# wjwei-handsome/wgatools

Hardware: AMD Instinct MI355X
Metric: paf_cigar_ops_per_s (paf2maf+stat) (higher is better)
Workload: dtype u8

## Files before the change

wgatools_amd/csrc/wga_kernels_k2s.h:

```cpp
#ifndef WGA_KERNELS_K2S_H
#define WGA_KERNELS_K2S_H

#include "wga_kernels.h"

#define WGA_S_FIFO 320u
#define WGA_S_MAX_TILE_COLS (1ull << 24)
#define WGA_S_MAX_JOB_TILES 32u
#define WGA_S_SKIP 0x100u
#define WGA_S_U 4u
#define WGA_S_WAVE_BYTES ((WGA_S_FIFO + 4u) * 8u + 1024u + 1024u + 256u + 272u + 16u)
#ifndef WGA_AUTO_LONG_VARIANT
#define WGA_AUTO_LONG_VARIANT 3
#endif

__global__ __launch_bounds__(256) void k_stream_mark_rec(u32 n, const wga_rec_desc* recs, const u64* op_off, u64 t_fa_bytes,
                                                         u64 q_fa_bytes, u8* tile_flag) {
  const u32 r = blockIdx.x * 256u + threadIdx.x;
  if (r >= n) return;
  const wga_rec_desc d = recs[r];
  const bool inside = d.t_src_off >= 32ull && d.t_src_off + d.t_src_len + 32ull <= t_fa_bytes && d.q_src_off >= 32ull &&
                      d.q_src_off + d.q_src_len + 32ull <= q_fa_bytes;
  if ((d.neg & 0xEull) == 0ull && inside) return;
  const u64 a = op_off[r], b = op_off[r + 1];
  if (b <= a) return;
// ... 29 lines not shown
  d.q_src_len = q_src_len ? q_src_len[r] : 0ull;
  d.I_total = cs.i + cs.s;
  d.D_total = cs.d;
  d.L = cs.mx + cs.d;
  const bool clean = !q_src_len || d.q_src_len == cs.mx + cs.i + cs.s;
  const bool inside = !q_src_off || (d.q_src_off >= 32ull && d.q_src_off + d.q_src_len + 32ull <= q_fa_bytes);
  d.neg = (strand_neg[r] != 0 ? 1u : 0u) | (clean ? 0u : 8u);
  out[r] = d;
  if (clean && inside) return;
  const u64 a = op_off[r], b = op_off[r + 1];
  if (b <= a) return;
  for (u64 t = a / WGA_TILE; t <= (b - 1) / WGA_TILE; t++) tile_flag[t] = 1;
}

__device__ __forceinline__ u32 comp4s(u32 x, u32* bad) {
  const u32 sel = x & 0x07070707u;
  const u32 fold = byte_perm(0x474EFF54u, 0x43FF41FFu, sel);
  const u32 comp = byte_perm(0x434E0D41u, 0x47FF54FFu, sel);
  *bad = (x & 0xDFDFDFDFu) ^ fold;
  return comp | (x & 0x20202020u);
}

#define WGA_S_NOINLINE __forceinline__
__device__ WGA_S_NOINLINE void stream_store_bytes(u8* p, u32 o0, u32 o1, u32 o2, u32 o3, int lo, int hi) {
#pragma clang loop vectorize(disable) unroll(disable)
  for (int j = lo; j < hi; j++) {
    const u32 wj = j < 4 ? o0 : j < 8 ? o1 : j < 12 ? o2 : o3;
    p[j] = (u8)(wj >> (8 * (j & 3)));
  }
}
__device__ WGA_S_NOINLINE void stream_report_bad(u64* bad_base_pos, u32 b0, u32 b1, u32 b2, u32 b3, int lo, int hi, u32 Cl,
                                                 i64 Kseg, const u32* fifo, u32 k, u32 nf, u32 adj) {
#pragma clang loop vectorize(disable) unroll(disable)
  for (int j = lo; j < hi; j++) {
    const u32 bw = j < 4 ? b0 : j < 8 ? b1 : j < 12 ? b2 : b3;
    if (((bw >> (8 * (j & 3))) & 0xFFu) == 0u) continue;
    const u32 cj = Cl + (u32)j;
    u32 ad = adj;
    if (fifo) {
      u32 i = k - 1u;
      while (i + 1u < nf && (int)(fifo[2u * (i + 1u)] - cj) <= 0) i++;
      ad = fifo[2u * (i + 1u) + 1u];
    }
    atomicMin(bad_base_pos, (u64)((i64)(u64)(cj - ad) + Kseg));
  }
}
// ... 55 lines not shown
    u32 n_new = nf;
    if (lane == 0u) {
      u32 w = e0;
      for (u32 r = e0; r < nf; r++) {
        const u32 gs = s_fifo[2u * r], cu = s_fifo[2u * r + 1u];
        const bool dup = w > e0 && s_fifo[2u * (w - 1u)] == gs && (int)(cu - s_fifo[2u * (w - 1u) + 1u]) <= 0 &&
                         (int)(s_fifo[2u * (r + 1u) + 1u] - cu) <= 0;
        if (!dup) {
          s_fifo[2u * w] = gs;
          s_fifo[2u * w + 1u] = cu;
          w++;
        }
      }
      for (u32 k = 0; k < 3u; k++) {
        s_fifo[2u * (w + k)] = s_fifo[2u * (nf + k)];
        s_fifo[2u * (w + k) + 1u] = s_fifo[2u * (nf + k) + 1u];
      }
      n_new = w;
    }
    nf = wave_get_u32(n_new, 0);
    WGA_WAVE_SYNC();
  };

  for (;;) {
    {
      const u32 lim = bnd ? C_b : C_known;
      const bool all = bnd || fin;
      while ((int)(lim - pos) > 0) {
        if (TCOORD && (int)(C_min - pos) > 0) {
          const u32 to = (int)(lim - C_min) > 0 ? C_min : lim;
          u32 c;
          do {
            const u32 idx = e0 + lane < nf ? e0 + lane : nf;
            c = (u32)__popcll(__ballot(idx < nf && (int)(s_fifo[2u * idx] - to) < 0));
            e0 += c;
          } while (c == 64u);
          pos = to;
          continue;
        }
        u8* const A = dst_seg + pos;
        const u32 mis = (u32)(u64)A & 1023u;
        u8* const B = A - mis;
        const u32 room = WGA_S_U * 1024u - mis;
        if (!all && (lim - pos) < room) break;
        const u32 Cs = pos;
        u32 Ce = (lim - pos) < room ? lim : pos + room;
        const u32 Cl0 = Cs - mis;
        if (e0 + 255u < nf) {
          const u32 g255 = WGA_UNI32(s_fifo[2u * (e0 + 255u)]);
          if ((int)(g255 - Ce) < 0) Ce = Cl0 + ((g255 - Cl0) & ~15u);
          if (MODE == WGA_S_PSEUDO && (int)(Ce - Cs) < 16) {
            fifo_dedupe();
            continue;
          }
        }

        s_T[lane] = 0u;
        WGA_WAVE_SYNC();
        u32 nE = 0;
        {
          u32 base = e0, c;
          do {
            const u32 idx = base + lane < nf ? base + lane : nf;
            const u32 gsr = s_fifo[2u * idx] - Cl0;
            const bool in = gsr < Ce - Cl0;
            c = (u32)__popcll(__ballot(in));
            if (in) atomicAdd(&s_T[(gsr >> 4) & 63u], 1u << (8u * (gsr >> 10)));
            base += c;
            nE += c;
          } while (c == 64u);
        }
        WGA_WAVE_SYNC();
        const u32 tw = s_T[lane];
        WGA_WAVE_SYNC();
        const u32 tinc = wave_incl_scan_u32(tw);
        const u32 texc = tinc - tw;
        const u32 ttot = wave_last_u32(tinc);

        u32 kbase = e0;
        u32 qn = 0, rpk = 0, cls = 0;
        u32 adjv[WGA_S_U];
        const u32 wsp = Ce - Cs - 16u, asp = Ce - Cs + 15u;
        const bool any16 = (Ce - Cs) >= 16u;
        u32 qcum = 0;
#pragma unroll
        for (u32 u = 0; u < WGA_S_U; u++) {
          const u32 cnt = (tw >> (8u * u)) & 255u;
          const u32 k = kbase + ((texc >> (8u * u)) & 255u);
          kbase += (ttot >> (8u * u)) & 255u;
          const u32 Cl = Cl0 + 1024u * u + 16u * lane;
          const bool whole = any16 && (Cl - Cs) <= wsp, active = (Cl + 15u - Cs) < asp;
          const u32x4_a1 fe = *(const u32x4_a1*)(s_fifo + 2u * (k - 1u));
          const int rel0 = (int)(fe[0] + stream_glen<MODE>(fe[1], fe[3]) - Cl);
          const bool quiet = whole && cnt == 0u;
          const bool plain = quiet && rel0 <= 0;
          const bool dashes = quiet && rel0 >= 16;
          const bool flagged = active && !(plain || dashes);
          adjv[u] = fe[3];
          cls |= ((plain ? 1u : 0u) | (dashes ? 2u : 0u) | (flagged ? 4u : 0u) | (SYM ? (fe[1] & 1u) << 3 : 0u)) << (4u * u);
          const u64 m = __ballot(flagged);
          if (flagged) {
            const u32 r = qn + lane_rank(m, lane);
            s_q[r & 255u] = (k << 8) | (u << 6) | lane;
            rpk |= (r & 255u) << (8u * u);
          }
          qcum |= (qn > 255u ? 255u : qn) << (8u * u);
          qn += (u32)__popcll(m);
        }
        if (qn > 64u) {
          u32 keep = 1u;
#pragma unroll
          for (u32 u = 2; u <= WGA_S_U; u++) {
            const u32 upto = u == WGA_S_U ? qn : (qcum >> (8u * u)) & 255u;
            const bool sat = u < WGA_S_U && ((qcum >> (8u * u)) & 255u) == 255u;
            if (upto <= 64u && !sat) keep = u;
          }
          const u32 Cn = Cl0 + 1024u * keep;
          if ((int)(Cn - Ce) < 0) Ce = Cn;
          qn = keep == WGA_S_U ? qn : (qcum >> (8u * keep)) & 255u;
          nE = 0;
#pragma unroll
          for (u32 u = 0; u < WGA_S_U; u++)
            if (u < keep) nE += (ttot >> (8u * u)) & 255u;
        }
        const BufRsrc dbuf = buf_make(B, WGA_S_U * 1024u);

        WGA_WAVE_SYNC();
        if (lane < qn) {
          const u32 ent = s_q[lane];
          const u32 k = ent >> 8, Cl = Cl0 + 16u * (ent & 255u);
          int lo = (int)(Cs - Cl), hi = (int)(Ce - Cl);
          lo = lo < 0 ? 0 : (lo > 16 ? 16 : lo);
          hi = hi > 16 ? 16 : (hi < 0 ? 0 : hi);
          const u32x4_a1 ea = *(const u32x4_a1*)(s_fifo + 2u * (k - 1u));
          const u32x4_a1 eb = *(const u32x4_a1*)(s_fifo + 2u * (k + 1u));
          const u32 gs0 = ea[0], cu0 = ea[1], gs1 = ea[2], cu1 = ea[3], gs2 = eb[0], cu2 = eb[1];
          int a1 = (int)(gs0 + stream_glen<MODE>(cu0, cu1) - Cl);
          a1 = a1 < lo ? lo : (a1 > hi ? hi : a1);
          int b1 = (int)(gs1 - Cl);
          b1 = b1 < a1 ? a1 : (b1 > hi ? hi : b1);
          const u32 gl1 = stream_glen<MODE>(cu1, cu2);
          int e1 = gl1 >= 16u ? 16 : b1 + (int)gl1;
          e1 = e1 > hi ? hi : e1;
          bool more = (int)(gs2 - Cl) < hi;
          u32 W0[4], W1[4];
          if (!SYM) {
            buf_load16(sbuf, b1 > a1 ? (rc ? S32 - Cl + cu1 : S32 + Cl - cu1) : WGA_BUF_OOB, W0);
            buf_load16(sbuf, hi > e1 ? (rc ? S32 - Cl + cu2 : S32 + Cl - cu2) : WGA_BUF_OOB, W1);
          }
          const u32x4_a16 La = s_lm[a1], Lb = s_lm[b1], Le = s_lm[e1];
          u32 o[4], bad[4] = {0u, 0u, 0u, 0u};
#pragma unroll
          for (int d = 0; d < 4; d++) {
            if (SYM) {
              o[d] = bfi_b32(La[d], stream_symbol(cu0), bfi_b32(Le[d] & ~Lb[d], stream_symbol(cu1), 0x31313131u));
              continue;
            }
            u32 cp;
            if (rc)
              cp = comp4s(bfi_b32(Lb[d], bswap32(W0[3 - d]), bswap32(W1[3 - d])), &bad[d]);
            else
              cp = bfi_b32(Lb[d], W0[d], W1[d]);
            const u32 md = La[d] | (Le[d] & ~Lb[d]);
            o[d] = bfi_b32(md, 0x2D2D2D2Du, cp);
            bad[d] &= ~md;
          }
          u32 ie = k + 1u;
          while (more) {
            const u32 gsi = s_fifo[2u * ie], cui = s_fifo[2u * ie + 1u], gsn = s_fifo[2u * ie + 2u], cun = s_fifo[2u * ie + 3u];
            const int b = (int)(gsi - Cl);
            const u32 len = stream_glen<MODE>(cui, cun);
            const int e = len >= (u32)(hi - b) ? hi : b + (int)len;
            u32 W[4];
            if (SYM)
              W[0] = W[1] = W[2] = W[3] = 0x31313131u;
            else
              buf_load16(sbuf, rc ? S32 - Cl + cun : S32 + Cl - cun, W);
            const u32x4_a16 Mb = s_lm[b], Me = s_lm[e];
#pragma unroll
            for (int d = 0; d < 4; d++) {
              u32 x = W[d], bw = 0u;
              if (rc) x = comp4s(bswap32(W[3 - d]), &bw);
              if (SYM)
                o[d] = bfi_b32(Mb[d], o[d], bfi_b32(Me[d], stream_symbol(cui), x));
              else
                o[d] = bfi_b32(Mb[d], o[d], bfi_b32(Me[d], 0x2D2D2D2Du, x));
              bad[d] = (bad[d] & Mb[d]) | (bw & ~Me[d]);
            }
            ie++;
            more = (int)(gsn - Cl) < hi;
          }
          if (rc && (bad[0] | bad[1] | bad[2] | bad[3]) != 0u)
            stream_report_bad((u64*)&a.diag[rec].bad_base_pos, bad[0], bad[1], bad[2], bad[3], lo, hi, Cl, (i64)s_k[0], s_fifo, k, nf, 0u);
          const u32x4_a16 ov = {o[0], o[1], o[2], o[3]};
          s_P[lane] = ov;
        }
        WGA_WAVE_SYNC();

        u32 dat[WGA_S_U][4];
        const u32 wsp2 = Ce - Cs - 16u;
#pragma unroll
        for (u32 u = 0; u < WGA_S_U; u++) {
          const u32 Cl = Cl0 + 1024u * u + 16u * lane;
          const u32 c = (cls >> (4u * u)) & 15u;
          if (SYM) {
            dat[u][0] = dat[u][1] = dat[u][2] = dat[u][3] = (c & 2u) ? ((c & 8u) ? 0x2D2D2D2Du : 0x30303030u) : 0x31313131u;
            continue;
          }
          dat[u][0] = dat[u][1] = dat[u][2] = dat[u][3] = (c & 2u) ? 0x2D2D2D2Du : 0u;
          if ((c & 1u) && (int)(Cl - Ce) < 0) buf_load16(sbuf, rc ? S32 - Cl + adjv[u] : S32 + Cl - adjv[u], dat[u]);
        }
        if (rc) {
#pragma unroll
          for (u32 u = 0; u < WGA_S_U; u++) {
            u32 bad[4], x[4];
#pragma unroll
            for (int d = 0; d < 4; d++) x[d] = comp4s(bswap32(dat[u][3 - d]), &bad[d]);
#pragma unroll
            for (int d = 0; d < 4; d++) dat[u][d] = x[d];
            const u32 Cl = Cl0 + 1024u * u + 16u * lane;
            const bool pb = ((cls >> (4u * u)) & 1u) != 0u && (int)(Cl - Ce) < 0 && (bad[0] | bad[1] | bad[2] | bad[3]) != 0u;
            if (__ballot(pb)) {
              if (pb)
                stream_report_bad((u64*)&a.diag[rec].bad_base_pos, bad[0], bad[1], bad[2], bad[3], 0, 16, Cl, (i64)s_k[0], nullptr, 0u, 0u,
                                  adjv[u]);
            }
          }
        }
#pragma unroll
        for (u32 u = 0; u < WGA_S_U; u++) {
          const u32 Cl = Cl0 + 1024u * u + 16u * lane;
          const bool queued = ((cls >> (4u * u)) & 4u) != 0u && (int)(Cl - Ce) < 0;
          if (queued) {
            const u32x4_a16 pv = s_P[(rpk >> (8u * u)) & 255u];
            dat[u][0] = pv[0];
            dat[u][1] = pv[1];
            dat[u][2] = pv[2];
            dat[u][3] = pv[3];
          }
          const bool whole = (Ce - Cs) >= 16u && (Cl - Cs) <= wsp2;
          buf_store16_stream(dbuf, whole ? 1024u * u + 16u * lane : WGA_BUF_OOB, dat[u]);
          if (queued && !whole) {
            int lo = (int)(Cs - Cl), hi = (int)(Ce - Cl);
            lo = lo < 0 ? 0 : lo;
            hi = hi > 16 ? 16 : hi;
            stream_store_bytes(B + 1024u * u + lane * 16u, dat[u][0], dat[u][1], dat[u][2], dat[u][3], lo, hi);
          }
        }
        WGA_WAVE_SYNC();
        e0 += nE;
        pos = Ce;
      }
      fin = false;
    }

    if (bnd || !live) {
      const bool sw = bnd;
      u64 row_off, src_off, src_len, x_a, sb;
      bool neg;
      u32 C_a, cum_a;
      if (bnd) {
        const u64 bnd_op = job_lo + re;
        u64 ren;
        do {
          rec++;
          ren = WGA_UNI64(a.op_off[rec + 1]);
        } while (ren <= bnd_op);
        re = ren - job_lo > (u64)q_end ? q_end : (u32)(ren - job_lo);
        const wga_rec_desc* const rd = a.recs + rec;
        row_off = WGA_UNI64(QROW ? rd->q_row_off : rd->t_row_off);
        src_off = WGA_UNI64(QROW ? rd->q_src_off : rd->t_src_off);
        src_len = WGA_UNI64(QROW ? rd->q_src_len : rd->t_src_len);
        neg = (WGA_UNI64(rd->neg) & 1ull) != 0ull;
        x_a = 0;
        sb = 0;
        C_a = C_b;
        cum_a = cum_b;
        if (TCOORD) {
          const u64 skip = WGA_UNI64(rd->t_src_len);
          C_min = C_a + (u32)(skip < 0x40000000ull ? skip : 0x40000000ull);
        }
      } else {
        while (t < t1 && (WGA_UNI32(a.tdesc[t].neg) & WGA_S_SKIP)) t++;
        if (t >= t1) break;
        const wga_tile_desc* const td = a.tdesc + t;
        const u64 tile_start = t * WGA_TILE;
        q = (u32)(tile_start - job_lo);
        WGA_WAVE_SYNC();
        C_known = cum_known = 0u;
        pos = 0u;
        nf = 1u;
        e0 = 1u;
        if (lane < 4u) {
          s_fifo[2u * lane] = 0u;
          s_fifo[2u * lane + 1u] = 0u;
        }
        rec = WGA_UNI32(td->rec);
        const u64 ren = WGA_UNI64(td->re), rs = WGA_UNI64(td->rs);
        re = ren - job_lo > (u64)q_end ? q_end : (u32)(ren - job_lo);
        const bool cont = rs < tile_start;
        const u64 b_mx = cont ? WGA_UNI64(td->b_mx) : 0ull, b_i = cont ? WGA_UNI64(td->b_i) : 0ull,
                  b_d = cont ? WGA_UNI64(td->b_d) : 0ull;
        row_off = WGA_UNI64(QROW ? td->q_row_off : td->t_row_off);
        src_off = WGA_UNI64(QROW ? td->q_src_off : td->t_src_off);
        src_len = WGA_UNI64(QROW ? td->q_src_len : td->t_src_len);
        neg = (WGA_UNI32(td->neg) & 1u) != 0u;
        x_a = TCOORD ? b_mx + b_d : b_mx + b_i + b_d;
        sb = QROW ? b_mx + b_i : b_mx + b_d;
        C_a = cum_a = 0u;
        if (TCOORD) {
          const u64 skip = WGA_UNI64(td->t_src_len);
          const u64 ahead = skip > x_a ? skip - x_a : 0ull;
          C_min = (u32)(ahead < 0x40000000ull ? ahead : 0x40000000ull);
        }
        buf_load16(obuf, q * 4u + lane * 16u, own);
        live = true;
      }
      dst_seg = (u8*)((u64)a.out + row_off + x_a - (u64)C_a);
      rc = QROW && !SYM && neg;
      const u32 adv = C_a - cum_a;
      u64 base;
      if (rc) {
        const u64 top = src_off + src_len;
        const u64 hiB = top > sb ? top - sb : 0ull;
        base = hiB > 0x60000000ull ? hiB - 0x60000000ull : 0ull;
        S32 = (u32)(top - base) - 16u - (u32)sb + adv;
      } else {
        const u64 loB = src_off + sb;
        base = loB > 64ull ? loB - 64ull : 0ull;
        S32 = (u32)(loB - base) - adv;
      }
      base = base > fa_bytes ? fa_bytes : base;
      {
        const u64 left = fa_bytes - base;
        sbuf = buf_make(fa + base, left > 0xFFFFFFF0ull ? 0xFFFFFFF0u : (u32)left);
      }
      if (lane == 0u) s_k[0] = (u64)((i64)sb - (i64)(u64)adv);
      WGA_WAVE_SYNC();
      bnd = false;
      if (sw && re < q_hi) {
        const u32 kb = re - q_lo, e = kb & 3u;
        u32 vl = xl0, vg = xg0;
#pragma unroll
        for (u32 i = 0; i < 3u; i++) {
          const bool valid = q_lo + 4u * lane + i < q_hi && i < e;
          const u32 len = valid ? ow[i] >> 4 : 0u, code = ow[i] & 15u;
          vl += len & bit_mask(COL_MASK, code);
          vg += (len & bit_mask(GAP_MASK, code)) - (len & bit_mask(SKIP_MASK, code));
        }
        C_b = wave_get_u32_dyn(vl, kb >> 2);
        cum_b = wave_get_u32_dyn(vg, kb >> 2);
        bnd = true;
      }
      continue;
    }

    if (q >= q_end) {
      if (pos != C_known) {
        fin = true;
        continue;
      }
      break;
    }
    if ((q & (WGA_TILE - 1u)) == 0u) {
      t = (job_lo + q) / WGA_TILE;
      if (WGA_UNI32(a.tdesc[t].neg) & WGA_S_SKIP) {
        if (pos != C_known) {
          fin = true;
          continue;
        }
        live = false;
        t++;
        continue;
      }
    }
    if (e0 > 1u) {
      const u32 from = e0 - 1u, count = nf + 3u - from;
      for (u32 i0 = 0; i0 < count; i0 += 64u) {
        const u32 i = i0 + lane;
        u64 v = 0;
        if (i < count) v = *(const u64*)(s_fifo + 2u * (from + i));
        WGA_WAVE_SYNC();
        if (i < count) *(u64*)(s_fifo + 2u * i) = v;
        WGA_WAVE_SYNC();
      }
      nf -= from;
      e0 = 1u;
    }
    if (nf + 256u > WGA_S_FIFO) {
      fin = true;
      if (pos != C_known) continue;
      fin = false;
      if (MODE == WGA_S_PSEUDO) {
        fifo_dedupe();
        if (nf + 256u > WGA_S_FIFO) break;
      }
    }
    q_lo = q;
    q_hi = q + 256u < q_end ? q + 256u : q_end;
    q = q_hi;
    ow[0] = own[0], ow[1] = own[1], ow[2] = own[2], ow[3] = own[3];
    buf_load16(obuf, q_hi < q_end ? q_hi * 4u + lane * 16u : WGA_BUF_OOB, own);
    u32 l[4], g[4], sl = 0, sg = 0, sc = 0;
#pragma unroll
    for (int e = 0; e < 4; e++) {
      const bool valid = q_lo + 4u * lane + (u32)e < q_hi;
      const u32 len = valid ? ow[e] >> 4 : 0u, code = ow[e] & 15u;
      l[e] = len & bit_mask(COL_MASK, code);
      g[e] = (len & bit_mask(GAP_MASK, code)) - (len & bit_mask(SKIP_MASK, code));
      sl += l[e];
      sg += g[e];
      sc += g[e] != 0u ? 1u : 0u;
    }
    const u32 il = wave_incl_scan_u32(sl), ig = wave_incl_scan_u32(sg), ic = wave_incl_scan_u32(sc);
    xl0 = C_known + il - sl;
    xg0 = cum_known + ig - sg;
    {
      u32 xl = xl0, xg = xg0, xc = nf + ic - sc;
#pragma unroll
      for (int e = 0; e < 4; e++) {
        if (g[e] != 0u) {
          s_fifo[2u * xc] = xl;
          s_fifo[2u * xc + 1u] = SYM ? (xg << 1) | (bit_mask(0x404u, ow[e] & 15u) & 1u) : xg;
          xc++;
          xg += g[e];
        }
        xl += l[e];
      }
    }
    C_known += wave_last_u32(il);
    cum_known += wave_last_u32(ig);
    nf += wave_last_u32(ic);
    if (lane < 3u) {
      s_fifo[2u * (nf + lane)] = C_known;
      s_fifo[2u * (nf + lane) + 1u] = SYM ? cum_known << 1 : cum_known;
    }
    WGA_WAVE_SYNC();
    if (re < q_hi) {
      const u32 kb = re - q_lo, e = kb & 3u;
      u32 vl = xl0, vg = xg0;
#pragma unroll
      for (u32 i = 0; i < 3u; i++) {
        const bool valid = q_lo + 4u * lane + i < q_hi && i < e;
        const u32 len = valid ? ow[i] >> 4 : 0u, code = ow[i] & 15u;
        vl += len & bit_mask(COL_MASK, code);
        vg += (len & bit_mask(GAP_MASK, code)) - (len & bit_mask(SKIP_MASK, code));
      }
      C_b = wave_get_u32_dyn(vl, kb >> 2);
      cum_b = wave_get_u32_dyn(vg, kb >> 2);
      bnd = true;
    }
  }
}

__device__ __forceinline__ u64 xcd_job_of_block() {
  const u32 nb = gridDim.x, b = blockIdx.x, x = b & 7u, q = nb >> 3, r = nb & 7u;
  return (u64)(x * q + (x < r ? x : r) + (b >> 3));
}

__device__ __forceinline__ void expand_stream(const ExpandArgs& a) {
  __shared__ u32x4_a16 s_mem[2u * WGA_S_WAVE_BYTES / 16u];
  const u32 lane = threadIdx.x & 63u, wave = WGA_WAVE_ID(threadIdx.x);
  const u64 nt = (a.n_ops + WGA_TILE - 1) / WGA_TILE;
  const u64 job = xcd_job_of_block();
  const u64 t0 = job * a.job_tiles;
  if (t0 >= nt) return;
  const u64 t1 = t0 + a.job_tiles < nt ? t0 + a.job_tiles : nt;
  u8* const lds = (u8*)s_mem + wave * WGA_S_WAVE_BYTES;
  if (wave == 0u)
    stream_row<0>(a, lds, lane, t0, t1);
  else
    stream_row<1>(a, lds, lane, t0, t1);
}
// ... 22 lines not shown
```

Baseline: 80.16 billion.

## Software-pipeline stream expand loop: plan next chunk while current chunk's loads fly

Restructures the wave's streaming expand loop into a two-stage state machine. Each iteration issues the source loads and builds the queued gap words for the previously planned chunk, then plans the next chunk (fifo histogram, classification, queue build) before doing the complement/merge and store of the current one. The aim is to hide global-load latency behind the planning work and LDS scans. The cost is extra carried state in registers, with a risk of register pressure or reduced occupancy, plus more complex control flow for refilling ops and switching records.

```diff
diff --git a/wgatools_amd/csrc/wga_kernels_k2s.h b/wgatools_amd/csrc/wga_kernels_k2s.h
--- a/wgatools_amd/csrc/wga_kernels_k2s.h
+++ b/wgatools_amd/csrc/wga_kernels_k2s.h
@@ -75,6 +75,11 @@
 }
 
 #define WGA_S_NOINLINE __forceinline__
+#ifdef WGA_EMU
+#define WGA_S_ARRIVED4(v) ((void)0)
+#else
+#define WGA_S_ARRIVED4(v) asm volatile("" : "+v"((v)[0]), "+v"((v)[1]), "+v"((v)[2]), "+v"((v)[3]))
+#endif
 __device__ WGA_S_NOINLINE void stream_store_bytes(u8* p, u32 o0, u32 o1, u32 o2, u32 o3, int lo, int hi) {
 #pragma clang loop vectorize(disable) unroll(disable)
   for (int j = lo; j < hi; j++) {
@@ -176,323 +181,325 @@
     WGA_WAVE_SYNC();
   };
 
+  u32 st = 0;
+  u32 p_Cs = 0, p_Ce = 0, p_Cl0 = 0, p_qn = 0, p_cls = 0, p_rpk = 0, p_adj[WGA_S_U] = {0, 0, 0, 0};
+  u8* p_B = nullptr;
+
   for (;;) {
-    {
-      const u32 lim = bnd ? C_b : C_known;
-      const bool all = bnd || fin;
-      while ((int)(lim - pos) > 0) {
-        if (TCOORD && (int)(C_min - pos) > 0) {
-          const u32 to = (int)(lim - C_min) > 0 ? C_min : lim;
-          u32 c;
-          do {
-            const u32 idx = e0 + lane < nf ? e0 + lane : nf;
-            c = (u32)__popcll(__ballot(idx < nf && (int)(s_fifo[2u * idx] - to) < 0));
-            e0 += c;
-          } while (c == 64u);
-          pos = to;
+    const bool step = st == 1u;
+    const bool idle = st == 0u;
+    const u32 Cs = p_Cs, Ce = p_Ce, Cl0 = p_Cl0, qn = p_qn, cls = p_cls, rpk = p_rpk;
+    const u32 adjv[WGA_S_U] = {p_adj[0], p_adj[1], p_adj[2], p_adj[3]};
+    u8* const B = p_B;
+    u32 dat[WGA_S_U][4] = {{0, 0, 0, 0}, {0, 0, 0, 0}, {0, 0, 0, 0}, {0, 0, 0, 0}};
+
+    if (step) {
+      WGA_WAVE_SYNC();
+      if (lane < qn) {
+        const u32 ent = s_q[lane];
+        const u32 k = ent >> 8, Cl = Cl0 + 16u * (ent & 255u);
+        int lo = (int)(Cs - Cl), hi = (int)(Ce - Cl);
+        lo = lo < 0 ? 0 : (lo > 16 ? 16 : lo);
+        hi = hi > 16 ? 16 : (hi < 0 ? 0 : hi);
+        const u32x4_a1 ea = *(const u32x4_a1*)(s_fifo + 2u * (k - 1u));
+        const u32x4_a1 eb = *(const u32x4_a1*)(s_fifo + 2u * (k + 1u));
+        const u32 gs0 = ea[0], cu0 = ea[1], gs1 = ea[2], cu1 = ea[3], gs2 = eb[0], cu2 = eb[1];
+        int a1 = (int)(gs0 + stream_glen<MODE>(cu0, cu1) - Cl);
+        a1 = a1 < lo ? lo : (a1 > hi ? hi : a1);
+        int b1 = (int)(gs1 - Cl);
+        b1 = b1 < a1 ? a1 : (b1 > hi ? hi : b1);
+        const u32 gl1 = stream_glen<MODE>(cu1, cu2);
+        int e1 = gl1 >= 16u ? 16 : b1 + (int)gl1;
+        e1 = e1 > hi ? hi : e1;
+        bool more = (int)(gs2 - Cl) < hi;
+        u32 W0[4], W1[4];
+        if (!SYM) {
+          buf_load16(sbuf, b1 > a1 ? (rc ? S32 - Cl + cu1 : S32 + Cl - cu1) : WGA_BUF_OOB, W0);
+          buf_load16(sbuf, hi > e1 ? (rc ? S32 - Cl + cu2 : S32 + Cl - cu2) : WGA_BUF_OOB, W1);
+        }
+        const u32x4_a16 La = s_lm[a1], Lb = s_lm[b1], Le = s_lm[e1];
+        u32 o[4], bad[4] = {0u, 0u, 0u, 0u};
+#pragma unroll
+        for (int d = 0; d < 4; d++) {
+          if (SYM) {
+            o[d] = bfi_b32(La[d], stream_symbol(cu0), bfi_b32(Le[d] & ~Lb[d], stream_symbol(cu1), 0x31313131u));
+            continue;
+          }
+          u32 cp;
+          if (rc)
+            cp = comp4s(bfi_b32(Lb[d], bswap32(W0[3 - d]), bswap32(W1[3 - d])), &bad[d]);
+          else
+            cp = bfi_b32(Lb[d], W0[d], W1[d]);
+          const u32 md = La[d] | (Le[d] & ~Lb[d]);
+          o[d] = bfi_b32(md, 0x2D2D2D2Du, cp);
+          bad[d] &= ~md;
+        }
+        u32 ie = k + 1u;
+        while (more) {
+          const u32 gsi = s_fifo[2u * ie], cui = s_fifo[2u * ie + 1u], gsn = s_fifo[2u * ie + 2u], cun = s_fifo[2u * ie + 3u];
+          const int b = (int)(gsi - Cl);
+          const u32 len = stream_glen<MODE>(cui, cun);
+          const int e = len >= (u32)(hi - b) ? hi : b + (int)len;
+          u32 W[4];
+          if (SYM)
+            W[0] = W[1] = W[2] = W[3] = 0x31313131u;
+          else
+            buf_load16(sbuf, rc ? S32 - Cl + cun : S32 + Cl - cun, W);
+          const u32x4_a16 Mb = s_lm[b], Me = s_lm[e];
+#pragma unroll
+          for (int d = 0; d < 4; d++) {
+            u32 x = W[d], bw = 0u;
+            if (rc) x = comp4s(bswap32(W[3 - d]), &bw);
+            if (SYM)
+              o[d] = bfi_b32(Mb[d], o[d], bfi_b32(Me[d], stream_symbol(cui), x));
+            else
+              o[d] = bfi_b32(Mb[d], o[d], bfi_b32(Me[d], 0x2D2D2D2Du, x));
+            bad[d] = (bad[d] & Mb[d]) | (bw & ~Me[d]);
+          }
+          ie++;
+          more = (int)(gsn - Cl) < hi;
+        }
+        if (rc && (bad[0] | bad[1] | bad[2] | bad[3]) != 0u)
+          stream_report_bad((u64*)&a.diag[rec].bad_base_pos, bad[0], bad[1], bad[2], bad[3], lo, hi, Cl, (i64)s_k[0], s_fifo, k, nf, 0u);
+        const u32x4_a16 ov = {o[0], o[1], o[2], o[3]};
+        s_P[lane] = ov;
+      }
+      WGA_WAVE_SYNC();
+
+      WGA_S_ARRIVED4(own);
+#pragma unroll
+      for (u32 u = 0; u < WGA_S_U; u++) {
+        const u32 Cl = Cl0 + 1024u * u + 16u * lane;
+        const u32 c = (cls >> (4u * u)) & 15u;
+        if (SYM) {
+          dat[u][0] = dat[u][1] = dat[u][2] = dat[u][3] = (c & 2u) ? ((c & 8u) ? 0x2D2D2D2Du : 0x30303030u) : 0x31313131u;
           continue;
         }
-        u8* const A = dst_seg + pos;
-        const u32 mis = (u32)(u64)A & 1023u;
-        u8* const B = A - mis;
-        const u32 room = WGA_S_U * 1024u - mis;
-        if (!all && (lim - pos) < room) break;
-        const u32 Cs = pos;
-        u32 Ce = (lim - pos) < room ? lim : pos + room;
-        const u32 Cl0 = Cs - mis;
-        if (e0 + 255u < nf) {
-          const u32 g255 = WGA_UNI32(s_fifo[2u * (e0 + 255u)]);
-          if ((int)(g255 - Ce) < 0) Ce = Cl0 + ((g255 - Cl0) & ~15u);
-          if (MODE == WGA_S_PSEUDO && (int)(Ce - Cs) < 16) {
+        dat[u][0] = dat[u][1] = dat[u][2] = dat[u][3] = (c & 2u) ? 0x2D2D2D2Du : 0u;
+#ifdef WGA_S_ABL_FIXED_SRC
+        if ((c & 1u) && (int)(Cl - Ce) < 0) buf_load16(sbuf, 64u + 16u * lane, dat[u]);
+#else
+        if ((c & 1u) && (int)(Cl - Ce) < 0) buf_load16(sbuf, rc ? S32 - Cl + adjv[u] : S32 + Cl - adjv[u], dat[u]);
+#endif
+      }
+    }
+
+    bool take = false;
+    if (step) {
+      const u32 room = WGA_S_U * 1024u - ((u32)(u64)(dst_seg + pos) & 1023u);
+      take = !bnd && !fin && q < q_end && (q & (WGA_TILE - 1u)) != 0u && nf - e0 + 257u <= WGA_S_FIFO && (C_known - pos) < room &&
+             !(TCOORD && (int)(C_min - pos) > 0);
+    } else if (idle) {
+      bool done = false;
+      do {
+        fin = false;
+        if (bnd || !live) {
+          const bool sw = bnd;
+          u64 row_off, src_off, src_len, x_a, sb;
+          bool neg;
+          u32 C_a, cum_a;
+          if (bnd) {
+            const u64 bnd_op = job_lo + re;
+            u64 ren;
+            do {
+              rec++;
+              ren = WGA_UNI64(a.op_off[rec + 1]);
+            } while (ren <= bnd_op);
+            re = ren - job_lo > (u64)q_end ? q_end : (u32)(ren - job_lo);
+            const wga_rec_desc* const rd = a.recs + rec;
+            row_off = WGA_UNI64(QROW ? rd->q_row_off : rd->t_row_off);
+            src_off = WGA_UNI64(QROW ? rd->q_src_off : rd->t_src_off);
+            src_len = WGA_UNI64(QROW ? rd->q_src_len : rd->t_src_len);
+            neg = (WGA_UNI64(rd->neg) & 1ull) != 0ull;
+            x_a = 0;
+            sb = 0;
+            C_a = C_b;
+            cum_a = cum_b;
+            if (TCOORD) {
+              const u64 skip = WGA_UNI64(rd->t_src_len);
+              C_min = C_a + (u32)(skip < 0x40000000ull ? skip : 0x40000000ull);
+            }
+          } else {
+            while (t < t1 && (WGA_UNI32(a.tdesc[t].neg) & WGA_S_SKIP)) t++;
+            if (t >= t1) {
+              done = true;
+              break;
+            }
+            const wga_tile_desc* const td = a.tdesc + t;
+            const u64 tile_start = t * WGA_TILE;
+            q = (u32)(tile_start - job_lo);
+            WGA_WAVE_SYNC();
+            C_known = cum_known = 0u;
+            pos = 0u;
+            nf = 1u;
+            e0 = 1u;
+            if (lane < 4u) {
+              s_fifo[2u * lane] = 0u;
+              s_fifo[2u * lane + 1u] = 0u;
+            }
+            rec = WGA_UNI32(td->rec);
+            const u64 ren = WGA_UNI64(td->re), rs = WGA_UNI64(td->rs);
+            re = ren - job_lo > (u64)q_end ? q_end : (u32)(ren - job_lo);
+            const bool cont = rs < tile_start;
+            const u64 b_mx = cont ? WGA_UNI64(td->b_mx) : 0ull, b_i = cont ? WGA_UNI64(td->b_i) : 0ull,
+                      b_d = cont ? WGA_UNI64(td->b_d) : 0ull;
+            row_off = WGA_UNI64(QROW ? td->q_row_off : td->t_row_off);
+            src_off = WGA_UNI64(QROW ? td->q_src_off : td->t_src_off);
+            src_len = WGA_UNI64(QROW ? td->q_src_len : td->t_src_len);
+            neg = (WGA_UNI32(td->neg) & 1u) != 0u;
+            x_a = TCOORD ? b_mx + b_d : b_mx + b_i + b_d;
+            sb = QROW ? b_mx + b_i : b_mx + b_d;
+            C_a = cum_a = 0u;
+            if (TCOORD) {
+              const u64 skip = WGA_UNI64(td->t_src_len);
+              const u64 ahead = skip > x_a ? skip - x_a : 0ull;
+              C_min = (u32)(ahead < 0x40000000ull ? ahead : 0x40000000ull);
+            }
+            buf_load16(obuf, q * 4u + lane * 16u, own);
+            WGA_S_ARRIVED4(own);
+            live = true;
+          }
+          dst_seg = (u8*)((u64)a.out + row_off + x_a - (u64)C_a);
+          rc = QROW && !SYM && neg;
+          const u32 adv = C_a - cum_a;
+          u64 base;
+          if (rc) {
+            const u64 top = src_off + src_len;
+            const u64 hiB = top > sb ? top - sb : 0ull;
+            base = hiB > 0x60000000ull ? hiB - 0x60000000ull : 0ull;
+            S32 = (u32)(top - base) - 16u - (u32)sb + adv;
+          } else {
+            const u64 loB = src_off + sb;
+            base = loB > 64ull ? loB - 64ull : 0ull;
+            S32 = (u32)(loB - base) - adv;
+          }
+          base = base > fa_bytes ? fa_bytes : base;
+          {
+            const u64 left = fa_bytes - base;
+            sbuf = buf_make(fa + base, left > 0xFFFFFFF0ull ? 0xFFFFFFF0u : (u32)left);
+          }
+          if (lane == 0u) s_k[0] = (u64)((i64)sb - (i64)(u64)adv);
+          WGA_WAVE_SYNC();
+          bnd = false;
+          if (sw && re < q_hi) {
+            const u32 kb = re - q_lo, e = kb & 3u;
+            u32 vl = xl0, vg = xg0;
+#pragma unroll
+            for (u32 i = 0; i < 3u; i++) {
+              const bool valid = q_lo + 4u * lane + i < q_hi && i < e;
+              const u32 len = valid ? ow[i] >> 4 : 0u, code = ow[i] & 15u;
+              vl += len & bit_mask(COL_MASK, code);
+              vg += (len & bit_mask(GAP_MASK, code)) - (len & bit_mask(SKIP_MASK, code));
+            }
+            C_b = wave_get_u32_dyn(vl, kb >> 2);
+            cum_b = wave_get_u32_dyn(vg, kb >> 2);
+            bnd = true;
+          }
+          break;
+        }
+        if (q >= q_end) {
+          if (pos != C_known)
+            fin = true;
+          else
+            done = true;
+          break;
+        }
+        if ((q & (WGA_TILE - 1u)) == 0u) {
+          t = (job_lo + q) / WGA_TILE;
+          if (WGA_UNI32(a.tdesc[t].neg) & WGA_S_SKIP) {
+            if (pos != C_known) {
+              fin = true;
+            } else {
+              live = false;
+              t++;
+            }
+            break;
+          }
+        }
+        if (nf - e0 + 257u > WGA_S_FIFO) {
+          if (pos != C_known) {
+            fin = true;
+            break;
+          }
+          if (MODE == WGA_S_PSEUDO) {
             fifo_dedupe();
-            continue;
-          }
-        }
-
-        s_T[lane] = 0u;
-        WGA_WAVE_SYNC();
-        u32 nE = 0;
-        {
-          u32 base = e0, c;
-          do {
-            const u32 idx = base + lane < nf ? base + lane : nf;
-            const u32 gsr = s_fifo[2u * idx] - Cl0;
-            const bool in = gsr < Ce - Cl0;
-            c = (u32)__popcll(__ballot(in));
-            if (in) atomicAdd(&s_T[(gsr >> 4) & 63u], 1u << (8u * (gsr >> 10)));
-            base += c;
-            nE += c;
-          } while (c == 64u);
-        }
-        WGA_WAVE_SYNC();
-        const u32 tw = s_T[lane];
-        WGA_WAVE_SYNC();
-        const u32 tinc = wave_incl_scan_u32(tw);
-        const u32 texc = tinc - tw;
-        const u32 ttot = wave_last_u32(tinc);
-
-        u32 kbase = e0;
-        u32 qn = 0, rpk = 0, cls = 0;
-        u32 adjv[WGA_S_U];
-        const u32 wsp = Ce - Cs - 16u, asp = Ce - Cs + 15u;
-        const bool any16 = (Ce - Cs) >= 16u;
-        u32 qcum = 0;
-#pragma unroll
-        for (u32 u = 0; u < WGA_S_U; u++) {
-          const u32 cnt = (tw >> (8u * u)) & 255u;
-          const u32 k = kbase + ((texc >> (8u * u)) & 255u);
-          kbase += (ttot >> (8u * u)) & 255u;
-          const u32 Cl = Cl0 + 1024u * u + 16u * lane;
-          const bool whole = any16 && (Cl - Cs) <= wsp, active = (Cl + 15u - Cs) < asp;
-          const u32x4_a1 fe = *(const u32x4_a1*)(s_fifo + 2u * (k - 1u));
-          const int rel0 = (int)(fe[0] + stream_glen<MODE>(fe[1], fe[3]) - Cl);
-          const bool quiet = whole && cnt == 0u;
-          const bool plain = quiet && rel0 <= 0;
-          const bool dashes = quiet && rel0 >= 16;
-          const bool flagged = active && !(plain || dashes);
-          adjv[u] = fe[3];
-          cls |= ((plain ? 1u : 0u) | (dashes ? 2u : 0u) | (flagged ? 4u : 0u) | (SYM ? (fe[1] & 1u) << 3 : 0u)) << (4u * u);
-          const u64 m = __ballot(flagged);
-          if (flagged) {
-            const u32 r = qn + lane_rank(m, lane);
-            s_q[r & 255u] = (k << 8) | (u << 6) | lane;
-            rpk |= (r & 255u) << (8u * u);
-          }
-          qcum |= (qn > 255u ? 255u : qn) << (8u * u);
-          qn += (u32)__popcll(m);
-        }
-        if (qn > 64u) {
-          u32 keep = 1u;
-#pragma unroll
-          for (u32 u = 2; u <= WGA_S_U; u++) {
-            const u32 upto = u == WGA_S_U ? qn : (qcum >> (8u * u)) & 255u;
-            const bool sat = u < WGA_S_U && ((qcum >> (8u * u)) & 255u) == 255u;
-            if (upto <= 64u && !sat) keep = u;
-          }
-          const u32 Cn = Cl0 + 1024u * keep;
-          if ((int)(Cn - Ce) < 0) Ce = Cn;
-          qn = keep == WGA_S_U ? qn : (qcum >> (8u * keep)) & 255u;
-          nE = 0;
-#pragma unroll
-          for (u32 u = 0; u < WGA_S_U; u++)
-            if (u < keep) nE += (ttot >> (8u * u)) & 255u;
-        }
-        const BufRsrc dbuf = buf_make(B, WGA_S_U * 1024u);
-
-        WGA_WAVE_SYNC();
-        if (lane < qn) {
-          const u32 ent = s_q[lane];
-          const u32 k = ent >> 8, Cl = Cl0 + 16u * (ent & 255u);
-          int lo = (int)(Cs - Cl), hi = (int)(Ce - Cl);
-          lo = lo < 0 ? 0 : (lo > 16 ? 16 : lo);
-          hi = hi > 16 ? 16 : (hi < 0 ? 0 : hi);
-          const u32x4_a1 ea = *(const u32x4_a1*)(s_fifo + 2u * (k - 1u));
-          const u32x4_a1 eb = *(const u32x4_a1*)(s_fifo + 2u * (k + 1u));
-          const u32 gs0 = ea[0], cu0 = ea[1], gs1 = ea[2], cu1 = ea[3], gs2 = eb[0], cu2 = eb[1];
-          int a1 = (int)(gs0 + stream_glen<MODE>(cu0, cu1) - Cl);
-          a1 = a1 < lo ? lo : (a1 > hi ? hi : a1);
-          int b1 = (int)(gs1 - Cl);
-          b1 = b1 < a1 ? a1 : (b1 > hi ? hi : b1);
-          const u32 gl1 = stream_glen<MODE>(cu1, cu2);
-          int e1 = gl1 >= 16u ? 16 : b1 + (int)gl1;
-          e1 = e1 > hi ? hi : e1;
-          bool more = (int)(gs2 - Cl) < hi;
-          u32 W0[4], W1[4];
-          if (!SYM) {
-            buf_load16(sbuf, b1 > a1 ? (rc ? S32 - Cl + cu1 : S32 + Cl - cu1) : WGA_BUF_OOB, W0);
-            buf_load16(sbuf, hi > e1 ? (rc ? S32 - Cl + cu2 : S32 + Cl - cu2) : WGA_BUF_OOB, W1);
-          }
-          const u32x4_a16 La = s_lm[a1], Lb = s_lm[b1], Le = s_lm[e1];
-          u32 o[4], bad[4] = {0u, 0u, 0u, 0u};
-#pragma unroll
-          for (int d = 0; d < 4; d++) {
-            if (SYM) {
-              o[d] = bfi_b32(La[d], stream_symbol(cu0), bfi_b32(Le[d] & ~Lb[d], stream_symbol(cu1), 0x31313131u));
-              continue;
+            if (nf - e0 + 257u > WGA_S_FIFO) {
+              done = true;
+              break;
             }
-            u32 cp;
-            if (rc)
-              cp = comp4s(bfi_b32(Lb[d], bswap32(W0[3 - d]), bswap32(W1[3 - d])), &bad[d]);
-            else
-              cp = bfi_b32(Lb[d], W0[d], W1[d]);
-            const u32 md = La[d] | (Le[d] & ~Lb[d]);
-            o[d] = bfi_b32(md, 0x2D2D2D2Du, cp);
-            bad[d] &= ~md;
-          }
-          u32 ie = k + 1u;
-          while (more) {
-            const u32 gsi = s_fifo[2u * ie], cui = s_fifo[2u * ie + 1u], gsn = s_fifo[2u * ie + 2u], cun = s_fifo[2u * ie + 3u];
-            const int b = (int)(gsi - Cl);
-            const u32 len = stream_glen<MODE>(cui, cun);
-            const int e = len >= (u32)(hi - b) ? hi : b + (int)len;
-            u32 W[4];
-            if (SYM)
-              W[0] = W[1] = W[2] = W[3] = 0x31313131u;
-            else
-              buf_load16(sbuf, rc ? S32 - Cl + cun : S32 + Cl - cun, W);
-            const u32x4_a16 Mb = s_lm[b], Me = s_lm[e];
-#pragma unroll
-            for (int d = 0; d < 4; d++) {
-              u32 x = W[d], bw = 0u;
-              if (rc) x = comp4s(bswap32(W[3 - d]), &bw);
-              if (SYM)
-                o[d] = bfi_b32(Mb[d], o[d], bfi_b32(Me[d], stream_symbol(cui), x));
-              else
-                o[d] = bfi_b32(Mb[d], o[d], bfi_b32(Me[d], 0x2D2D2D2Du, x));
-              bad[d] = (bad[d] & Mb[d]) | (bw & ~Me[d]);
-            }
-            ie++;
-            more = (int)(gsn - Cl) < hi;
-          }
-          if (rc && (bad[0] | bad[1] | bad[2] | bad[3]) != 0u)
-            stream_report_bad((u64*)&a.diag[rec].bad_base_pos, bad[0], bad[1], bad[2], bad[3], lo, hi, Cl, (i64)s_k[0], s_fifo, k, nf, 0u);
-          const u32x4_a16 ov = {o[0], o[1], o[2], o[3]};
-          s_P[lane] = ov;
-        }
-        WGA_WAVE_SYNC();
-
-        u32 dat[WGA_S_U][4];
-        const u32 wsp2 = Ce - Cs - 16u;
-#pragma unroll
-        for (u32 u = 0; u < WGA_S_U; u++) {
-          const u32 Cl = Cl0 + 1024u * u + 16u * lane;
-          const u32 c = (cls >> (4u * u)) & 15u;
-          if (SYM) {
-            dat[u][0] = dat[u][1] = dat[u][2] = dat[u][3] = (c & 2u) ? ((c & 8u) ? 0x2D2D2D2Du : 0x30303030u) : 0x31313131u;
-            continue;
-          }
-          dat[u][0] = dat[u][1] = dat[u][2] = dat[u][3] = (c & 2u) ? 0x2D2D2D2Du : 0u;
-          if ((c & 1u) && (int)(Cl - Ce) < 0) buf_load16(sbuf, rc ? S32 - Cl + adjv[u] : S32 + Cl - adjv[u], dat[u]);
-        }
-        if (rc) {
-#pragma unroll
-          for (u32 u = 0; u < WGA_S_U; u++) {
-            u32 bad[4], x[4];
-#pragma unroll
-            for (int d = 0; d < 4; d++) x[d] = comp4s(bswap32(dat[u][3 - d]), &bad[d]);
-#pragma unroll
-            for (int d = 0; d < 4; d++) dat[u][d] = x[d];
-            const u32 Cl = Cl0 + 1024u * u + 16u * lane;
-            const bool pb = ((cls >> (4u * u)) & 1u) != 0u && (int)(Cl - Ce) < 0 && (bad[0] | bad[1] | bad[2] | bad[3]) != 0u;
-            if (__ballot(pb)) {
-              if (pb)
-                stream_report_bad((u64*)&a.diag[rec].bad_base_pos, bad[0], bad[1], bad[2], bad[3], 0, 16, Cl, (i64)s_k[0], nullptr, 0u, 0u,
-                                  adjv[u]);
-            }
-          }
-        }
-#pragma unroll
-        for (u32 u = 0; u < WGA_S_U; u++) {
-          const u32 Cl = Cl0 + 1024u * u + 16u * lane;
-          const bool queued = ((cls >> (4u * u)) & 4u) != 0u && (int)(Cl - Ce) < 0;
-          if (queued) {
-            const u32x4_a16 pv = s_P[(rpk >> (8u * u)) & 255u];
-            dat[u][0] = pv[0];
-            dat[u][1] = pv[1];
-            dat[u][2] = pv[2];
-            dat[u][3] = pv[3];
-          }
-          const bool whole = (Ce - Cs) >= 16u && (Cl - Cs) <= wsp2;
-          buf_store16_stream(dbuf, whole ? 1024u * u + 16u * lane : WGA_BUF_OOB, dat[u]);
-          if (queued && !whole) {
-            int lo = (int)(Cs - Cl), hi = (int)(Ce - Cl);
-            lo = lo < 0 ? 0 : lo;
-            hi = hi > 16 ? 16 : hi;
-            stream_store_bytes(B + 1024u * u + lane * 16u, dat[u][0], dat[u][1], dat[u][2], dat[u][3], lo, hi);
-          }
-        }
-        WGA_WAVE_SYNC();
-        e0 += nE;
-        pos = Ce;
-      }
-      fin = false;
+          }
+        }
+        take = true;
+      } while (false);
+      if (done) break;
     }
 
-    if (bnd || !live) {
-      const bool sw = bnd;
-      u64 row_off, src_off, src_len, x_a, sb;
-      bool neg;
-      u32 C_a, cum_a;
-      if (bnd) {
-        const u64 bnd_op = job_lo + re;
-        u64 ren;
-        do {
-          rec++;
-          ren = WGA_UNI64(a.op_off[rec + 1]);
-        } while (ren <= bnd_op);
-        re = ren - job_lo > (u64)q_end ? q_end : (u32)(ren - job_lo);
-        const wga_rec_desc* const rd = a.recs + rec;
-        row_off = WGA_UNI64(QROW ? rd->q_row_off : rd->t_row_off);
-        src_off = WGA_UNI64(QROW ? rd->q_src_off : rd->t_src_off);
-        src_len = WGA_UNI64(QROW ? rd->q_src_len : rd->t_src_len);
-        neg = (WGA_UNI64(rd->neg) & 1ull) != 0ull;
-        x_a = 0;
-        sb = 0;
-        C_a = C_b;
-        cum_a = cum_b;
-        if (TCOORD) {
-          const u64 skip = WGA_UNI64(rd->t_src_len);
-          C_min = C_a + (u32)(skip < 0x40000000ull ? skip : 0x40000000ull);
-        }
-      } else {
-        while (t < t1 && (WGA_UNI32(a.tdesc[t].neg) & WGA_S_SKIP)) t++;
-        if (t >= t1) break;
-        const wga_tile_desc* const td = a.tdesc + t;
-        const u64 tile_start = t * WGA_TILE;
-        q = (u32)(tile_start - job_lo);
-        WGA_WAVE_SYNC();
-        C_known = cum_known = 0u;
-        pos = 0u;
-        nf = 1u;
+    if (take) {
+      if (e0 > 1u) {
+        const u32 from = e0 - 1u, count = nf + 3u - from;
+        for (u32 i0 = 0; i0 < count; i0 += 64u) {
+          const u32 i = i0 + lane;
+          u64 v = 0;
+          if (i < count) v = *(const u64*)(s_fifo + 2u * (from + i));
+          WGA_WAVE_SYNC();
+          if (i < count) *(u64*)(s_fifo + 2u * i) = v;
+          WGA_WAVE_SYNC();
+        }
+        nf -= from;
         e0 = 1u;
-        if (lane < 4u) {
-          s_fifo[2u * lane] = 0u;
-          s_fifo[2u * lane + 1u] = 0u;
-        }
-        rec = WGA_UNI32(td->rec);
-        const u64 ren = WGA_UNI64(td->re), rs = WGA_UNI64(td->rs);
-        re = ren - job_lo > (u64)q_end ? q_end : (u32)(ren - job_lo);
-        const bool cont = rs < tile_start;
-        const u64 b_mx = cont ? WGA_UNI64(td->b_mx) : 0ull, b_i = cont ? WGA_UNI64(td->b_i) : 0ull,
-                  b_d = cont ? WGA_UNI64(td->b_d) : 0ull;
-        row_off = WGA_UNI64(QROW ? td->q_row_off : td->t_row_off);
-        src_off = WGA_UNI64(QROW ? td->q_src_off : td->t_src_off);
-        src_len = WGA_UNI64(QROW ? td->q_src_len : td->t_src_len);
-        neg = (WGA_UNI32(td->neg) & 1u) != 0u;
-        x_a = TCOORD ? b_mx + b_d : b_mx + b_i + b_d;
-        sb = QROW ? b_mx + b_i : b_mx + b_d;
-        C_a = cum_a = 0u;
-        if (TCOORD) {
-          const u64 skip = WGA_UNI64(td->t_src_len);
-          const u64 ahead = skip > x_a ? skip - x_a : 0ull;
-          C_min = (u32)(ahead < 0x40000000ull ? ahead : 0x40000000ull);
-        }
-        buf_load16(obuf, q * 4u + lane * 16u, own);
-        live = true;
-      }
-      dst_seg = (u8*)((u64)a.out + row_off + x_a - (u64)C_a);
-      rc = QROW && !SYM && neg;
-      const u32 adv = C_a - cum_a;
-      u64 base;
-      if (rc) {
-        const u64 top = src_off + src_len;
-        const u64 hiB = top > sb ? top - sb : 0ull;
-        base = hiB > 0x60000000ull ? hiB - 0x60000000ull : 0ull;
-        S32 = (u32)(top - base) - 16u - (u32)sb + adv;
-      } else {
-        const u64 loB = src_off + sb;
-        base = loB > 64ull ? loB - 64ull : 0ull;
-        S32 = (u32)(loB - base) - adv;
-      }
-      base = base > fa_bytes ? fa_bytes : base;
+      }
+      q_lo = q;
+      q_hi = q + 256u < q_end ? q + 256u : q_end;
+      q = q_hi;
+      ow[0] = own[0], ow[1] = own[1], ow[2] = own[2], ow[3] = own[3];
+      buf_load16(obuf, q_hi < q_end ? q_hi * 4u + lane * 16u : WGA_BUF_OOB, own);
+#ifdef WGA_S_ABL_INTAKE_TWICE
+#pragma clang loop unroll(disable)
+      for (u32 rep = 0; rep < 2u; rep++) {
+      asm volatile("" : "+v"(ow[0]), "+v"(ow[1]), "+v"(ow[2]), "+v"(ow[3]));
+#endif
+      u32 l[4], g[4], sl = 0, sg = 0, sc = 0;
+#pragma unroll
+      for (int e = 0; e < 4; e++) {
+        const bool valid = q_lo + 4u * lane + (u32)e < q_hi;
+        const u32 len = valid ? ow[e] >> 4 : 0u, code = ow[e] & 15u;
+        l[e] = len & bit_mask(COL_MASK, code);
+        g[e] = (len & bit_mask(GAP_MASK, code)) - (len & bit_mask(SKIP_MASK, code));
+        sl += l[e];
+        sg += g[e];
+        sc += g[e] != 0u ? 1u : 0u;
+      }
+      const u32 il = wave_incl_scan_u32(sl), ig = wave_incl_scan_u32(sg), ic = wave_incl_scan_u32(sc);
+      xl0 = C_known + il - sl;
+      xg0 = cum_known + ig - sg;
       {
-        const u64 left = fa_bytes - base;
-        sbuf = buf_make(fa + base, left > 0xFFFFFFF0ull ? 0xFFFFFFF0u : (u32)left);
-      }
-      if (lane == 0u) s_k[0] = (u64)((i64)sb - (i64)(u64)adv);
+        u32 xl = xl0, xg = xg0, xc = nf + ic - sc;
+#pragma unroll
+        for (int e = 0; e < 4; e++) {
+          if (g[e] != 0u) {
+            s_fifo[2u * xc] = xl;
+            s_fifo[2u * xc + 1u] = SYM ? (xg << 1) | (bit_mask(0x404u, ow[e] & 15u) & 1u) : xg;
+            xc++;
+            xg += g[e];
+          }
+          xl += l[e];
+        }
+      }
+#ifdef WGA_S_ABL_INTAKE_TWICE
+      if (rep == 0u) continue;
+#endif
+      C_known += wave_last_u32(il);
+      cum_known += wave_last_u32(ig);
+      nf += wave_last_u32(ic);
+      if (lane < 3u) {
+        s_fifo[2u * (nf + lane)] = C_known;
+        s_fifo[2u * (nf + lane) + 1u] = SYM ? cum_known << 1 : cum_known;
+      }
+#ifdef WGA_S_ABL_INTAKE_TWICE
+      }
+#endif
       WGA_WAVE_SYNC();
-      bnd = false;
-      if (sw && re < q_hi) {
+      if (re < q_hi) {
         const u32 kb = re - q_lo, e = kb & 3u;
         u32 vl = xl0, vg = xg0;
 #pragma unroll
@@ -506,103 +513,158 @@
         cum_b = wave_get_u32_dyn(vg, kb >> 2);
         bnd = true;
       }
-      continue;
     }
 
-    if (q >= q_end) {
-      if (pos != C_known) {
-        fin = true;
-        continue;
-      }
-      break;
-    }
-    if ((q & (WGA_TILE - 1u)) == 0u) {
-      t = (job_lo + q) / WGA_TILE;
-      if (WGA_UNI32(a.tdesc[t].neg) & WGA_S_SKIP) {
-        if (pos != C_known) {
-          fin = true;
-          continue;
-        }
-        live = false;
-        t++;
-        continue;
-      }
-    }
-    if (e0 > 1u) {
-      const u32 from = e0 - 1u, count = nf + 3u - from;
-      for (u32 i0 = 0; i0 < count; i0 += 64u) {
-        const u32 i = i0 + lane;
-        u64 v = 0;
-        if (i < count) v = *(const u64*)(s_fifo + 2u * (from + i));
-        WGA_WAVE_SYNC();
-        if (i < count) *(u64*)(s_fifo + 2u * i) = v;
-        WGA_WAVE_SYNC();
-      }
-      nf -= from;
-      e0 = 1u;
-    }
-    if (nf + 256u > WGA_S_FIFO) {
-      fin = true;
-      if (pos != C_known) continue;
-      fin = false;
-      if (MODE == WGA_S_PSEUDO) {
-        fifo_dedupe();
-        if (nf + 256u > WGA_S_FIFO) break;
-      }
-    }
-    q_lo = q;
-    q_hi = q + 256u < q_end ? q + 256u : q_end;
-    q = q_hi;
-    ow[0] = own[0], ow[1] = own[1], ow[2] = own[2], ow[3] = own[3];
-    buf_load16(obuf, q_hi < q_end ? q_hi * 4u + lane * 16u : WGA_BUF_OOB, own);
-    u32 l[4], g[4], sl = 0, sg = 0, sc = 0;
-#pragma unroll
-    for (int e = 0; e < 4; e++) {
-      const bool valid = q_lo + 4u * lane + (u32)e < q_hi;
-      const u32 len = valid ? ow[e] >> 4 : 0u, code = ow[e] & 15u;
-      l[e] = len & bit_mask(COL_MASK, code);
-      g[e] = (len & bit_mask(GAP_MASK, code)) - (len & bit_mask(SKIP_MASK, code));
-      sl += l[e];
-      sg += g[e];
-      sc += g[e] != 0u ? 1u : 0u;
-    }
-    const u32 il = wave_incl_scan_u32(sl), ig = wave_incl_scan_u32(sg), ic = wave_incl_scan_u32(sc);
-    xl0 = C_known + il - sl;
-    xg0 = cum_known + ig - sg;
-    {
-      u32 xl = xl0, xg = xg0, xc = nf + ic - sc;
-#pragma unroll
-      for (int e = 0; e < 4; e++) {
-        if (g[e] != 0u) {
-          s_fifo[2u * xc] = xl;
-          s_fifo[2u * xc + 1u] = SYM ? (xg << 1) | (bit_mask(0x404u, ow[e] & 15u) & 1u) : xg;
-          xc++;
-          xg += g[e];
-        }
-        xl += l[e];
-      }
-    }
-    C_known += wave_last_u32(il);
-    cum_known += wave_last_u32(ig);
-    nf += wave_last_u32(ic);
-    if (lane < 3u) {
-      s_fifo[2u * (nf + lane)] = C_known;
-      s_fifo[2u * (nf + lane) + 1u] = SYM ? cum_known << 1 : cum_known;
-    }
-    WGA_WAVE_SYNC();
-    if (re < q_hi) {
-      const u32 kb = re - q_lo, e = kb & 3u;
-      u32 vl = xl0, vg = xg0;
-#pragma unroll
-      for (u32 i = 0; i < 3u; i++) {
-        const bool valid = q_lo + 4u * lane + i < q_hi && i < e;
-        const u32 len = valid ? ow[i] >> 4 : 0u, code = ow[i] & 15u;
-        vl += len & bit_mask(COL_MASK, code);
-        vg += (len & bit_mask(GAP_MASK, code)) - (len & bit_mask(SKIP_MASK, code));
-      }
-      C_b = wave_get_u32_dyn(vl, kb >> 2);
-      cum_b = wave_get_u32_dyn(vg, kb >> 2);
-      bnd = true;
+    st = 0u;
+    do {
+      const u32 lim = bnd ? C_b : C_known;
+      const bool all = bnd || fin;
+      if ((int)(lim - pos) <= 0) break;
+      if (TCOORD && (int)(C_min - pos) > 0) {
+        st = 2u;
+        if (step) break;
+        const u32 to = (int)(lim - C_min) > 0 ? C_min : lim;
+        u32 c;
+        do {
+          const u32 idx = e0 + lane < nf ? e0 + lane : nf;
+          c = (u32)__popcll(__ballot(idx < nf && (int)(s_fifo[2u * idx] - to) < 0));
+          e0 += c;
+        } while (c == 64u);
+        pos = to;
+        break;
+      }
+      u8* const A = dst_seg + pos;
+      const u32 mis = (u32)(u64)A & 1023u;
+      const u32 room = WGA_S_U * 1024u - mis;
+      if (!all && (lim - pos) < room) break;
+      const u32 nCs = pos;
+      u32 nCe = (lim - pos) < room ? lim : pos + room;
+      const u32 nCl0 = nCs - mis;
+      if (e0 + 255u < nf) {
+        const u32 g255 = WGA_UNI32(s_fifo[2u * (e0 + 255u)]);
+        if ((int)(g255 - nCe) < 0) nCe = nCl0 + ((g255 - nCl0) & ~15u);
+        if (MODE == WGA_S_PSEUDO && (int)(nCe - nCs) < 16) {
+          st = 2u;
+          if (!step) fifo_dedupe();
+          break;
+        }
+      }
+
+      s_T[lane] = 0u;
+      WGA_WAVE_SYNC();
+      u32 nE = 0;
+      {
+        u32 base = e0, c;
+        do {
+          const u32 idx = base + lane < nf ? base + lane : nf;
+          const u32 gsr = s_fifo[2u * idx] - nCl0;
+          const bool in = gsr < nCe - nCl0;
+          c = (u32)__popcll(__ballot(in));
+          if (in) atomicAdd(&s_T[(gsr >> 4) & 63u], 1u << (8u * (gsr >> 10)));
+          base += c;
+          nE += c;
+        } while (c == 64u);
+      }
+      WGA_WAVE_SYNC();
+      const u32 tw = s_T[lane];
+      WGA_WAVE_SYNC();
+      const u32 tinc = wave_incl_scan_u32(tw);
+      const u32 texc = tinc - tw;
+      const u32 ttot = wave_last_u32(tinc);
+
+      u32 kbase = e0;
+      u32 nqn = 0, nrpk = 0, ncls = 0;
+      const u32 wsp = nCe - nCs - 16u, asp = nCe - nCs + 15u;
+      const bool any16 = (nCe - nCs) >= 16u;
+      u32 qcum = 0;
+#pragma unroll
+      for (u32 u = 0; u < WGA_S_U; u++) {
+        const u32 cnt = (tw >> (8u * u)) & 255u;
+        const u32 k = kbase + ((texc >> (8u * u)) & 255u);
+        kbase += (ttot >> (8u * u)) & 255u;
+        const u32 Cl = nCl0 + 1024u * u + 16u * lane;
+        const bool whole = any16 && (Cl - nCs) <= wsp, active = (Cl + 15u - nCs) < asp;
+        const u32x4_a1 fe = *(const u32x4_a1*)(s_fifo + 2u * (k - 1u));
+        const int rel0 = (int)(fe[0] + stream_glen<MODE>(fe[1], fe[3]) - Cl);
+        const bool quiet = whole && cnt == 0u;
+        const bool plain = quiet && rel0 <= 0;
+        const bool dashes = quiet && rel0 >= 16;
+        const bool flagged = active && !(plain || dashes);
+        p_adj[u] = fe[3];
+        ncls |= ((plain ? 1u : 0u) | (dashes ? 2u : 0u) | (flagged ? 4u : 0u) | (SYM ? (fe[1] & 1u) << 3 : 0u)) << (4u * u);
+        const u64 m = __ballot(flagged);
+        if (flagged) {
+          const u32 r = nqn + lane_rank(m, lane);
+          s_q[r & 255u] = (k << 8) | (u << 6) | lane;
+          nrpk |= (r & 255u) << (8u * u);
+        }
+        qcum |= (nqn > 255u ? 255u : nqn) << (8u * u);
+        nqn += (u32)__popcll(m);
+      }
+      if (nqn > 64u) {
+        u32 keep = 1u;
+#pragma unroll
+        for (u32 u = 2; u <= WGA_S_U; u++) {
+          const u32 upto = u == WGA_S_U ? nqn : (qcum >> (8u * u)) & 255u;
+          const bool sat = u < WGA_S_U && ((qcum >> (8u * u)) & 255u) == 255u;
+          if (upto <= 64u && !sat) keep = u;
+        }
+        const u32 Cn = nCl0 + 1024u * keep;
+        if ((int)(Cn - nCe) < 0) nCe = Cn;
+        nqn = keep == WGA_S_U ? nqn : (qcum >> (8u * keep)) & 255u;
+        nE = 0;
+#pragma unroll
+        for (u32 u = 0; u < WGA_S_U; u++)
+          if (u < keep) nE += (ttot >> (8u * u)) & 255u;
+      }
+      p_Cs = nCs, p_Ce = nCe, p_Cl0 = nCl0, p_qn = nqn, p_cls = ncls, p_rpk = nrpk;
+      p_B = A - mis;
+      e0 += nE;
+      pos = nCe;
+      st = 1u;
+    } while (false);
+
+    if (step) {
+      const BufRsrc dbuf = buf_make(B, WGA_S_U * 1024u);
+      const u32 wsp2 = Ce - Cs - 16u;
+      if (rc) {
+#pragma unroll
+        for (u32 u = 0; u < WGA_S_U; u++) {
+          u32 bad[4], x[4];
+#pragma unroll
+          for (int d = 0; d < 4; d++) x[d] = comp4s(bswap32(dat[u][3 - d]), &bad[d]);
+#pragma unroll
+          for (int d = 0; d < 4; d++) dat[u][d] = x[d];
+          const u32 Cl = Cl0 + 1024u * u + 16u * lane;
+          const bool pb = ((cls >> (4u * u)) & 1u) != 0u && (int)(Cl - Ce) < 0 && (bad[0] | bad[1] | bad[2] | bad[3]) != 0u;
+          if (__ballot(pb)) {
+            if (pb)
+              stream_report_bad((u64*)&a.diag[rec].bad_base_pos, bad[0], bad[1], bad[2], bad[3], 0, 16, Cl, (i64)s_k[0], nullptr, 0u, 0u,
+                                adjv[u]);
+          }
+        }
+      }
+#pragma unroll
+      for (u32 u = 0; u < WGA_S_U; u++) {
+        const u32 Cl = Cl0 + 1024u * u + 16u * lane;
+        const bool queued = ((cls >> (4u * u)) & 4u) != 0u && (int)(Cl - Ce) < 0;
+        if (queued) {
+          const u32x4_a16 pv = s_P[(rpk >> (8u * u)) & 255u];
+          dat[u][0] = pv[0];
+          dat[u][1] = pv[1];
+          dat[u][2] = pv[2];
+          dat[u][3] = pv[3];
+        }
+        const bool whole = (Ce - Cs) >= 16u && (Cl - Cs) <= wsp2;
+        buf_store16_stream(dbuf, whole ? 1024u * u + 16u * lane : WGA_BUF_OOB, dat[u]);
+        if (queued && !whole) {
+          int lo = (int)(Cs - Cl), hi = (int)(Ce - Cl);
+          lo = lo < 0 ? 0 : lo;
+          hi = hi > 16 ? 16 : hi;
+          stream_store_bytes(B + 1024u * u + lane * 16u, dat[u][0], dat[u][1], dat[u][2], dat[u][3], lo, hi);
+        }
+      }
+      WGA_WAVE_SYNC();
     }
   }
 }
```

Result: no change. 80.53 billion (median of 2 runs) (+0.5%).
